# MoFHeka/MeepoEmbedding

Hardware: AMD Instinct MI355X
Metric: key-lookups/sec (higher is better)
Workload: dtype int64 keys / fp32 rows (copy)

## Files before the change

### meepoembedding_amd/csrc/meepo_find.hip

```cpp
#include <hip/hip_runtime.h>
#include <hip/hip_ext.h>

#include <cmath>
#include <cstdlib>
#include <cstring>

#include "meepo_apply_part.h"


namespace mee {


template <int DIM4, int R, int NT>
__device__ __forceinline__ void find_span(const int64_t* __restrict__ tkeys, const f32x4* __restrict__ values, uint64_t nb,
                                          const int64_t* __restrict__ keys, uint64_t n, f32x4* __restrict__ out,
                                          uint8_t* __restrict__ found, float defv, uint32_t dim4_rt, uint32_t* hits,
                                          int64_t* __restrict__ slots_out, uint64_t wave, uint64_t n_waves, int64_t handle_tag = 0) {
    const int lane = threadIdx.x & 63, tile = lane >> 4, tl = lane & 15;
    const uint32_t dim4 = DIM4 ? DIM4 : dim4_rt;
    constexpr int KPW = 4 * R;
    const f32x4 def4 = {defv, defv, defv, defv};

    for (uint64_t base = wave * KPW; base < n; base += n_waves * KPW) {
        int64_t key[R];
        int64_t slot[R];
        uint64_t b[R];
        int64_t kb[R];
        bool inb[R], act[R];
        const int64_t kmine = (lane < KPW && base + lane < n) ? keys[base + lane] : kEmpty;
#pragma unroll
        for (int r = 0; r < R; ++r) {
            const uint64_t i = base + r * 4 + tile;
            inb[r] = i < n;
            key[r] = __shfl(kmine, r * 4 + tile);
            act[r] = inb[r] && !reserved_key(key[r]);
            if constexpr ((NT & 8) != 0) {
                inb[r] = act[r] = act[r] && found[i] == 0;
            }
            if constexpr ((NT & 128) != 0) {
                if (inb[r] && !act[r] && tl == 0 && found) found[i] = 1;
                inb[r] = act[r];
            }
        }
#pragma unroll
        for (int r = 0; r < R; ++r) {
            b[r] = bucket_of(key[r], nb);
            kb[r] = act[r] ? ((NT & 2) ? __builtin_nontemporal_load(&tkeys[b[r] * kW + tl]) : tkeys[b[r] * kW + tl]) : kEmpty;
        }
#pragma unroll
        for (int r = 0; r < R; ++r) slot[r] = tile_probe(tkeys, nb, key[r], act[r], b[r], kb[r], tile, tl);
        if constexpr ((NT & 16) != 0) {
#pragma unroll
            for (int r = 0; r < R; ++r)
                if (slot[r] >= 0 && tl == 0) atomicAdd(&hits[slot[r]], 1u);
        }
        if constexpr (DIM4 != 0) {
            constexpr int C = DIM4 / 16;
            f32x4 row[R][C];
            bool all_hit = true;
#pragma unroll
            for (int r = 0; r < R; ++r) all_hit = all_hit && inb[r] && slot[r] >= 0;
            if (__all(all_hit)) {
#pragma unroll
                for (int r = 0; r < R; ++r)
#pragma unroll
                    for (int c = 0; c < C; ++c)
                        row[r][c] = (NT & 1) ? __builtin_nontemporal_load(&values[(uint64_t)slot[r] * DIM4 + c * 16 + tl]) : values[(uint64_t)slot[r] * DIM4 + c * 16 + tl];
#pragma unroll
                for (int r = 0; r < R; ++r) {
                    const uint64_t i = base + r * 4 + tile;
#pragma unroll
                    for (int c = 0; c < C; ++c) {
                        if constexpr ((NT & 256) != 0) store_bf16x4<(NT & 4) != 0>(out, i * DIM4 + c * 16 + tl, row[r][c]);
                        else { if (NT & 4) out[i * DIM4 + c * 16 + tl] = row[r][c]; else __builtin_nontemporal_store(row[r][c], &out[i * DIM4 + c * 16 + tl]); }
                    }
                }
            } else {
#pragma unroll
                for (int r = 0; r < R; ++r)
#pragma unroll
                    for (int c = 0; c < C; ++c)
                        row[r][c] = slot[r] >= 0 ? ((NT & 1) ? __builtin_nontemporal_load(&values[(uint64_t)slot[r] * DIM4 + c * 16 + tl]) : values[(uint64_t)slot[r] * DIM4 + c * 16 + tl]) : def4;
#pragma unroll
                for (int r = 0; r < R; ++r) {
                    const uint64_t i = base + r * 4 + tile;
                    if (inb[r] && (!(NT & 8) || slot[r] >= 0)) {
#pragma unroll
                        for (int c = 0; c < C; ++c) {
                            if constexpr ((NT & 256) != 0) store_bf16x4<(NT & 4) != 0>(out, i * DIM4 + c * 16 + tl, row[r][c]);
                            else { if (NT & 4) out[i * DIM4 + c * 16 + tl] = row[r][c]; else __builtin_nontemporal_store(row[r][c], &out[i * DIM4 + c * 16 + tl]); }
                        }
                    }
                }
            }
        } else {
#pragma unroll
            for (int r = 0; r < R; ++r) {
                const uint64_t i = base + r * 4 + tile;
                if (inb[r] && (!(NT & 8) || slot[r] >= 0))
                    for (uint32_t c = tl; c < dim4; c += 16) {
                        if constexpr ((NT & 256) != 0) store_bf16x4<true>(out, i * dim4 + c, slot[r] >= 0 ? values[(uint64_t)slot[r] * dim4 + c] : def4);
                        else out[i * dim4 + c] = slot[r] >= 0 ? values[(uint64_t)slot[r] * dim4 + c] : def4;
                    }
            }
        }
        if constexpr ((NT & 64) != 0) {
            const int64_t mine = collect_slots(slot, lane);
            if (lane < KPW && base + lane < n) slots_out[base + lane] = mine >= 0 ? (mine | handle_tag) : mine;
        }
        if (found && !(NT & 32)) {
#pragma unroll
            for (int r = 0; r < R; ++r) {
                const uint64_t i0 = base + r * 4;
                if ((NT & (8 | 128)) == 0 && i0 + 4 <= n && (reinterpret_cast<uintptr_t>(found) & 3) == 0) {
                    const uint64_t m = __ballot(slot[r] >= 0);
                    const uint32_t w = (uint32_t)(m & 1) | ((uint32_t)((m >> 16) & 1) << 8) | ((uint32_t)((m >> 32) & 1) << 16) |
                                       ((uint32_t)((m >> 48) & 1) << 24);
                    if (lane == 0) *reinterpret_cast<uint32_t*>(found + i0) = w;
                } else {
                    const uint64_t i = i0 + tile;
                    if (inb[r] && tl == 0 && (!(NT & 8) || slot[r] >= 0)) found[i] = slot[r] >= 0;
                }
            }
        }
    }
}

template <int DIM4, int R, int NT>
__global__ __launch_bounds__(256) void find_kernel(const int64_t* __restrict__ tkeys, const f32x4* __restrict__ values,
                                                   uint64_t nb, const int64_t* __restrict__ keys, uint64_t n,
                                                   f32x4* __restrict__ out, uint8_t* __restrict__ found, float defv,
                                                   uint32_t dim4_rt, uint32_t* hits, int64_t* __restrict__ slots_out = nullptr, int64_t handle_tag = 0) {
    find_span<DIM4, R, NT>(tkeys, values, nb, keys, n, out, found, defv, dim4_rt, hits, slots_out,
                           (uint64_t)blockIdx.x * (blockDim.x >> 6) + (threadIdx.x >> 6), (uint64_t)gridDim.x * (blockDim.x >> 6), handle_tag);
}

constexpr int kFindPrepareThreads = 256;
constexpr int kFindPrepareR = 2;
template <int DIM4, int R, int NT>
__global__ __launch_bounds__(kFindPrepareThreads, 8) void find_prepare_kernel(const int64_t* __restrict__ tkeys, const f32x4* __restrict__ values, uint64_t nb,
                                                           const int64_t* __restrict__ keys, uint64_t n, f32x4* __restrict__ out,
                                                           uint8_t* __restrict__ found, float defv, uint32_t dim4_rt, int64_t* __restrict__ slots_out,
                                                           int64_t handle_tag, uint32_t part_blocks, uint32_t nbk_hash, uint32_t nbk, uint32_t per_block,
                                                           BucketScratch bk, uint32_t* status, OpCounters* op, uint32_t xcd_split) {
    extern __shared__ unsigned long long part_lds[];
    __shared__ unsigned long long part_wsum[kFindPrepareThreads / 64];
    if (blockIdx.x < part_blocks) {
        PartHot* hot = reinterpret_cast<PartHot*>(part_lds);
        sort_role<kFindPrepareThreads>(keys, (uint32_t)n, nbk_hash, nbk, per_block, blockIdx.x, part_blocks, bk, status, op, reinterpret_cast<uint32_t*>(hot + 1), part_wsum, hot, true, xcd_split);
        return;
    }
    find_span<DIM4, R, NT>(tkeys, values, nb, keys, n, out, found, defv, dim4_rt, nullptr, slots_out,
                           (uint64_t)(blockIdx.x - part_blocks) * (blockDim.x >> 6) + (threadIdx.x >> 6), (uint64_t)(gridDim.x - part_blocks) * (blockDim.x >> 6),
                           handle_tag);
}

constexpr int kMaxFindRequests = 16;
struct FindMany {
    const int64_t* keys[kMaxFindRequests];
    f32x4* out[kMaxFindRequests];
    uint8_t* found[kMaxFindRequests];
    uint64_t n[kMaxFindRequests];
    uint32_t first_block[kMaxFindRequests + 1];
    uint32_t count;
};
template <int DIM4, int R, int NT>
__global__ __launch_bounds__(256) void find_many_kernel(const int64_t* __restrict__ tkeys, const f32x4* __restrict__ values, uint64_t nb,
// ... 351 lines not shown
                pooled_bwd_positions<DIM4, U, C, GROUPED>(tkeys, values, nb, capacity, dim4, kv, pos, inb, wv, handles, handle_tag, member,
                                                          tile, tl, def4, g, grads, weight_grads);
            }
        }
    }
}

}

using namespace mee;

namespace mee {
static bool outputs_rotate(const mee_table* t, const void* d_out, uint64_t bytes) {
    mee_table* m = const_cast<mee_table*>(t);
    const uint64_t p = (uint64_t)(uintptr_t)d_out;
    const uint32_t head = __atomic_load_n(&m->out_ring_head, __ATOMIC_RELAXED);
    if (__atomic_load_n(&m->out_ring_ptr[(head + 7u) & 7u], __ATOMIC_RELAXED) == p) return false;
    const uint32_t slot = __atomic_fetch_add(&m->out_ring_head, 1u, __ATOMIC_RELAXED) & 7u;
    __atomic_store_n(&m->out_ring_ptr[slot], p, __ATOMIC_RELAXED);
    __atomic_store_n(&m->out_ring_bytes[slot], bytes, __ATOMIC_RELAXED);
    uint64_t seen[8], total = 0;
    int distinct = 0;
    for (int i = 0; i < 8; ++i) {
        const uint64_t q = __atomic_load_n(&m->out_ring_ptr[i], __ATOMIC_RELAXED);
        if (!q) continue;
        bool dup = false;
        for (int j = 0; j < distinct; ++j) dup = dup || seen[j] == q;
        if (dup) continue;
        seen[distinct++] = q;
        total += __atomic_load_n(&m->out_ring_bytes[i], __ATOMIC_RELAXED);
    }
    return distinct >= 2 && total > (64ull << 20);
}

template <class F> void with_pooled_shape(uint32_t dim4, size_t n, uint64_t n_bags, F&& f) {
    with_row_shape(dim4, [&](auto d4) {
        if (n / n_bags >= 12) f(d4, std::integral_constant<int, RowShape<d4>::pooled_unroll_1>{}, std::integral_constant<int, 1>{}, grid_for(n_bags, 4, 1u << 20));
        else f(d4, std::integral_constant<int, RowShape<d4>::pooled_unroll_4>{}, std::integral_constant<int, 4>{}, grid_for(n_bags, 16, 1u << 20));
    });
}

int find_plane(const mee_table* t, const float* plane, float miss_value, const int64_t* d_keys, size_t n, float* d_out,
               uint8_t* d_found, void* stream, FindPath path) {
    if (n == 0) return MEE_OK;
    DeviceGuard g(t->device);
    hipStream_t st = as_stream(stream);
    const unsigned fblock = t->find_block == 64 || t->find_block == 128 ? (unsigned)t->find_block : 256u;
    const bool bf16 = path.out_dtype == MEE_DTYPE_BF16;
    const uint64_t out_bytes = (uint64_t)n * t->dim * (bf16 ? 2 : 4);
    const int nt = path.nt >= 0 ? path.nt : t->find_nt >= 0 ? (t->find_nt & 7)
                 : (out_bytes <= kCachedOutputBytes && !outputs_rotate(t, d_out, out_bytes) ? 4 : 0);
    if (path.kind == FindPath::Missing || path.kind == FindPath::CountedMissing) {
        with_value<3, 1>(path.kind == FindPath::CountedMissing ? 3 : 1, [&](auto flags) {
            find_missing_kernel<flags><<<grid_for(n, 256, 8192), 256, 0, st>>>(t->keys, (const float4*)plane, t->nb, t->dim4, d_keys, n, (float4*)d_out, d_found, t->hits);
        });
    } else if (bf16) with_row_shape(t->dim4, [&](auto d4) {
        constexpr int D4 = d4;
        constexpr int R = RowShape<D4>::rows_per_tile;
        const unsigned grid = grid_for(n, (fblock / 64u) * 4u * (unsigned)R, t->find_grid_cap > 0 ? (unsigned)t->find_grid_cap : (1u << 22));
        auto find = [&](auto ntc, int64_t* slots_out, int64_t tag) {
            find_kernel<D4, R, ntc><<<grid, fblock, 0, st>>>(t->keys, (const f32x4*)plane, t->nb, d_keys, n, (f32x4*)d_out, d_found, miss_value, t->dim4, nullptr, slots_out, tag);
        };
        if (path.kind == FindPath::Located) {
            const bool cached_out = t->find_nt >= 0 && (t->find_nt & 4);
            with_value<256 + 68, 256 + 64>(cached_out ? 256 + 68 : 256 + 64, [&](auto ntc) { find(ntc, path.slots_out, handle_tag_of(t)); });
        } else if (path.kind == FindPath::SkipPadding) {
            with_value<256 + 132, 256 + 128>(nt & 4 ? 256 + 132 : 256 + 128, [&](auto ntc) { find(ntc, nullptr, 0); });
        } else {
            with_value<256, 257, 258, 259, 260, 261, 262, 263>(256 | nt, [&](auto ntc) { find(ntc, nullptr, 0); });
        }
    });
    else with_row_shape(t->dim4, [&](auto d4) {
        constexpr int D4 = d4;
        int R = t->find_rounds > 0 ? t->find_rounds : RowShape<D4>::rows_per_tile;
        if (D4 != 16 && R > 4) R = 4;
        if (D4 != 16 && D4 != 32 && R > 2) R = 2;
        R = R >= 8 ? 8 : R >= 4 ? 4 : R >= 2 ? 2 : 1;
        const unsigned grid = grid_for(n, (fblock / 64u) * 4u * (unsigned)R, t->find_grid_cap > 0 ? (unsigned)t->find_grid_cap : (1u << 22));
        auto find = [&](auto rr, auto ntc, unsigned grid_x, unsigned block, uint32_t* hits = nullptr, int64_t* slots_out = nullptr, int64_t tag = 0) {
            find_kernel<D4, rr, ntc><<<grid_x, block, 0, st>>>(t->keys, (const f32x4*)plane, t->nb, d_keys, n, (f32x4*)d_out, d_found, miss_value, t->dim4, hits, slots_out, tag);
        };
        if (path.kind == FindPath::SkipPadding) {
            with_value<2, 1>(R >= 2 ? 2 : 1, [&](auto rr) { with_value<132, 128>(nt & 4 ? 132 : 128, [&](auto ntc) { find(rr, ntc, grid, 256); }); });
        } else if (path.kind == FindPath::Located) {
// ... 29 lines not shown
    if ((flags & MEE_FIND_STREAM_STORES) && (flags & MEE_FIND_CACHED_STORES))
        return fail(MEE_ERR_INVALID_ARG, "%s: MEE_FIND_STREAM_STORES and MEE_FIND_CACHED_STORES exclude each other", name);
    if (flags == MEE_FIND_DEFAULT) return find_plane(t, t->values, t->default_value, d_keys, n, (float*)d_out, d_found, stream, {FindPath::Plain, nullptr, -1, out_dtype});
    const uint64_t out_bytes = (uint64_t)n * t->dim * (out_dtype == MEE_DTYPE_BF16 ? 2 : 4);
    const bool cached_out = (flags & MEE_FIND_CACHED_STORES) ||
                            (!(flags & MEE_FIND_STREAM_STORES) && out_bytes <= kCachedOutputBytes && !outputs_rotate(t, d_out, out_bytes));
    const int nt = (flags & MEE_FIND_STREAM_ROWS ? 1 : 0) | (flags & MEE_FIND_STREAM_BUCKETS ? 2 : 0) | (cached_out ? 4 : 0);
    return find_plane(t, t->values, t->default_value, d_keys, n, (float*)d_out, d_found, stream, {FindPath::Plain, nullptr, nt, out_dtype});
}

int mee_find(const mee_table* t, const int64_t* d_keys, size_t n, float* d_out, uint8_t* d_found, void* stream) {
    MEE_RANGE("mee_find");
    if (!t || (n && (!d_keys || !d_out))) return fail(MEE_ERR_INVALID_ARG, "mee_find: null argument");
    return find_plane(t, t->values, t->default_value, d_keys, n, d_out, d_found, stream);
}

int mee_find_ex(const mee_table* t, const int64_t* d_keys, size_t n, float* d_out, uint8_t* d_found, uint32_t flags, void* stream) {
    MEE_RANGE("mee_find_ex");
    return find_hinted(t, d_keys, n, d_out, d_found, flags, MEE_DTYPE_F32, stream, "mee_find_ex");
}

int mee_find_as(const mee_table* t, const int64_t* d_keys, size_t n, void* d_out, uint32_t out_dtype, uint8_t* d_found, uint32_t flags, void* stream) {
    MEE_RANGE("mee_find_as");
    return find_hinted(t, d_keys, n, d_out, d_found, flags, out_dtype, stream, "mee_find_as");
}

}
namespace mee {
int find_skip_padding(const mee_table* t, const int64_t* d_keys, size_t n, void* d_out, uint8_t* d_found, void* stream, uint32_t out_dtype) {
    if (!t || (n && (!d_keys || !d_out || !d_found))) return fail(MEE_ERR_INVALID_ARG, "find_skip_padding: null argument");
    if (int rc = check_out_dtype(d_out, out_dtype, "find_skip_padding")) return rc;
    return find_plane(t, t->values, t->default_value, d_keys, n, (float*)d_out, d_found, stream, {FindPath::SkipPadding, nullptr, -1, out_dtype});
}
}
extern "C" {

int mee_find_located(const mee_table* t, const int64_t* d_keys, size_t n, float* d_out, uint8_t* d_found, int64_t* d_slots_out, void* stream) {
    MEE_RANGE("mee_find_located");
    if (!t || (n && (!d_keys || !d_out || !d_slots_out))) return fail(MEE_ERR_INVALID_ARG, "mee_find_located: null argument");
    return find_plane(t, t->values, t->default_value, d_keys, n, d_out, d_found, stream, {FindPath::Located, d_slots_out});
}
int mee_find_located_as(const mee_table* t, const int64_t* d_keys, size_t n, void* d_out, uint32_t out_dtype, uint8_t* d_found, int64_t* d_slots_out, void* stream) {
    MEE_RANGE("mee_find_located_as");
    if (!t || (n && (!d_keys || !d_out || !d_slots_out))) return fail(MEE_ERR_INVALID_ARG, "mee_find_located_as: null argument");
    if (int rc = check_out_dtype(d_out, out_dtype, "mee_find_located_as")) return rc;
    return find_plane(t, t->values, t->default_value, d_keys, n, (float*)d_out, d_found, stream, {FindPath::Located, d_slots_out, -1, out_dtype});
}

int mee_find_many(const mee_table* t, const mee_find_request* reqs, uint32_t count, void* stream) {
    MEE_RANGE("mee_find_many");
    if (!t || !reqs) return fail(MEE_ERR_INVALID_ARG, "mee_find_many: null argument");
    if (count == 0) return MEE_OK;
    if (count > (uint32_t)kMaxFindRequests) return fail(MEE_ERR_INVALID_ARG, "mee_find_many: %u requests (at most %d per call)", count, kMaxFindRequests);
    FindMany m{};
    const int R = with_row_shape(t->dim4, [](auto d4) { return RowShape<d4>::rows_per_tile; });
    uint64_t blocks = 0, out_bytes = 0;
    uint32_t used = 0;
    for (uint32_t q = 0; q < count; ++q) {
        if (reqs[q].n == 0) continue;
        if (!reqs[q].d_keys || !reqs[q].d_out) return fail(MEE_ERR_INVALID_ARG, "mee_find_many: request %u has a null buffer", q);
        m.keys[used] = reqs[q].d_keys; m.out[used] = (f32x4*)reqs[q].d_out; m.found[used] = reqs[q].d_found; m.n[used] = reqs[q].n;
        m.first_block[used] = (uint32_t)blocks;
        blocks += (reqs[q].n + 16ull * R - 1) / (16ull * R);
        out_bytes += (uint64_t)reqs[q].n * t->dim * 4;
        ++used;
    }
// ... 207 lines not shown
```

### meepoembedding_amd/csrc/meepo_host.h

```cpp
#pragma once
#include <hip/hip_runtime.h>
#include <cstdarg>
#include <cstdio>
#include <type_traits>

#include "../../include/meepo_embedding.h"

namespace mee {

char* last_error_buf();

inline int fail(int code, const char* fmt, ...) {
    va_list ap;
    va_start(ap, fmt);
    vsnprintf(last_error_buf(), 512, fmt, ap);
    va_end(ap);
    return code;
}

#define MEE_HIP(expr)                                                                                     \
    do {                                                                                                  \
        hipError_t e_ = (expr);                                                                           \
        if (e_ != hipSuccess)                                                                             \
            return ::mee::fail(e_ == hipErrorOutOfMemory ? MEE_ERR_OUT_OF_MEMORY : MEE_ERR_HIP,           \
// ... 19 lines not shown
    OpRange& operator=(const OpRange&) = delete;
};
#define MEE_RANGE(name) ::mee::OpRange mee_range_(name)

struct DeviceGuard {
    int prev = -1;
    bool switched = false;
    hipError_t err = hipSuccess;
    explicit DeviceGuard(int device) {
        err = hipGetDevice(&prev);
        if (err == hipSuccess && prev != device) { err = hipSetDevice(device); switched = (err == hipSuccess); }
    }
    ~DeviceGuard() { if (switched) (void)hipSetDevice(prev); }
};

struct TableView {
    int device;
    const int64_t* keys;
    const float* values;
    uint64_t nb;
    uint32_t dim, dim4;
    float default_value;
    uint64_t generation;
    float *s1, *s2;
    uint32_t optimizer;
    uint32_t initializer;
    float init_scale, init_acc;
    uint64_t init_seed;
    uint32_t* status;
    uint32_t* hits;
};
TableView table_view(const mee_table* t);
int find_skip_padding(const mee_table* t, const int64_t* d_keys, size_t n, void* d_out, uint8_t* d_found, void* stream, uint32_t out_dtype = MEE_DTYPE_F32);

struct GroupDesc {
    const int64_t* tkeys;
    float4* values;
    float4* s1;
    float4* s2;
    uint64_t nb;
    float defv;
    uint32_t pad;
};
struct GroupInit {
    uint64_t init_seed;
    uint32_t* status;
    uint32_t* hits;
    uint32_t initializer, optimizer;
    float init_scale, init_acc;
};
constexpr int kGroupSlotBits = 48;
constexpr uint32_t kMaxGroupTables = 1024;

inline unsigned grid_for(size_t work_items, unsigned per_block, unsigned cap) {
    size_t g = (work_items + per_block - 1) / per_block;
    if (g < 1) g = 1;
    if (g > cap) g = cap;
    return (unsigned)g;
}

constexpr uint64_t kCachedOutputBytes = 128ull << 20;

template <class F> decltype(auto) with_row_shape(uint32_t dim4, F&& f) {
    if (dim4 == 16) return f(std::integral_constant<int, 16>{});
    if (dim4 == 32) return f(std::integral_constant<int, 32>{});
    return f(std::integral_constant<int, 0>{});
// ... 33 lines not shown
```

### meepoembedding_amd/csrc/meepo_sharded.hip

```cpp
#include <hip/hip_runtime.h>
#include <rccl/rccl.h>

#include <dlfcn.h>

#include <atomic>
#include <cmath>
#include <cstdlib>
#include <cstring>
#include <mutex>
#include <new>
#include <mutex>
#include <unordered_set>
#include <vector>

#include "meepo_device.h"
#include "meepo_host.h"

namespace mee {

struct RcclApi {
    void* handle = nullptr;
    ncclResult_t (*GetUniqueId)(ncclUniqueId*) = nullptr;
    ncclResult_t (*CommInitRank)(ncclComm_t*, int, ncclUniqueId, int) = nullptr;
    ncclResult_t (*CommDestroy)(ncclComm_t) = nullptr;
// ... 40 lines not shown
    });
    return api.handle ? &api : nullptr;
}
static const char* rccl_load_error() {
    (void)rccl_api();
    return rccl_state().error[0] ? rccl_state().error : "RCCL could not be loaded (librccl.so.1 not found or incomplete)";
}

#define MEE_NCCL(api, expr)                                                                                        \
    do {                                                                                                           \
        ncclResult_t r_ = (expr);                                                                                  \
        if (r_ != ncclSuccess)                                                                                     \
            return ::mee::fail(MEE_ERR_RCCL, "%s failed: %s (%s:%d)", #expr, (api)->GetErrorString(r_), __FILE__, __LINE__); \
    } while (0)

__device__ __forceinline__ uint64_t seg_base(const uint64_t* __restrict__ counts, uint32_t p) {
    uint64_t b = 0;
    for (uint32_t q = 0; q < p; ++q) b += counts[q];
    return b;
}

__global__ __launch_bounds__(256) void shard_pad_keys_kernel(const int64_t* __restrict__ send_keys, const uint64_t* __restrict__ counts,
                                                             uint64_t cap, int64_t* __restrict__ pad, uint32_t* status) {
    const uint32_t p = blockIdx.y;
    const uint64_t cnt = counts[p], take = cnt < cap ? cnt : cap, b0 = seg_base(counts, p);
    int64_t* __restrict__ dst = pad + (uint64_t)p * cap;
    for (uint64_t j = blockIdx.x * (uint64_t)blockDim.x + threadIdx.x; j < cap; j += (uint64_t)gridDim.x * blockDim.x)
        dst[j] = j < take ? send_keys[b0 + j] : kEmpty;
    if (cnt > cap && blockIdx.x == 0 && threadIdx.x == 0) atomicOr(status, 1u);
}

__global__ __launch_bounds__(256) void shard_pack_rows_kernel(const float4* __restrict__ rows, const int64_t* __restrict__ perm,
                                                              const uint64_t* __restrict__ counts, uint64_t cap ,
                                                              uint32_t dim4, float4* __restrict__ dst) {
    const int lane = threadIdx.x & 63, tile = lane >> 4, tl = lane & 15;
    const uint32_t p = blockIdx.y;
    const uint64_t cnt = counts[p], take = (cap && cnt > cap) ? cap : cnt, b0 = seg_base(counts, p);
    const uint64_t off = cap ? (uint64_t)p * cap : b0;
    const uint64_t wave = (uint64_t)blockIdx.x * (blockDim.x >> 6) + (threadIdx.x >> 6), n_waves = (uint64_t)gridDim.x * (blockDim.x >> 6);
    for (uint64_t j0 = wave * 4; j0 < take; j0 += n_waves * 4) {
        const uint64_t j = j0 + tile;
        if (j >= take) continue;
        const uint64_t src = (uint64_t)perm[b0 + j] * dim4;
        for (uint32_t c = tl; c < dim4; c += 16) dst[(off + j) * dim4 + c] = rows[src + c];
    }
}

template <bool BF16> struct RowGroup { using type = float4; };
template <> struct RowGroup<true> { using type = u32x2; };
template <bool BF16>
__global__ __launch_bounds__(256) void shard_return_kernel(const typename RowGroup<BF16>::type* __restrict__ back_rows, const uint8_t* __restrict__ back_found,
                                                           const int64_t* __restrict__ perm, const uint64_t* __restrict__ counts,
                                                           uint64_t cap , uint32_t dim4, typename RowGroup<BF16>::type* __restrict__ out,
                                                           uint8_t* __restrict__ found, float defv, const int64_t* __restrict__ send_keys) {
    const int lane = threadIdx.x & 63, tile = lane >> 4, tl = lane & 15;
    const uint32_t p = blockIdx.y;
    const uint64_t cnt = counts[p], take = (cap && cnt > cap) ? cap : cnt, b0 = seg_base(counts, p);
    const uint64_t off = cap ? (uint64_t)p * cap : b0;
    const uint64_t wave = (uint64_t)blockIdx.x * (blockDim.x >> 6) + (threadIdx.x >> 6), n_waves = (uint64_t)gridDim.x * (blockDim.x >> 6);
    typename RowGroup<BF16>::type def4;
    if constexpr (BF16) def4 = bf16x4_of(defv, defv, defv, defv); else def4 = make_float4(defv, defv, defv, defv);
    for (uint64_t j0 = wave * 4; j0 < cnt; j0 += n_waves * 4) {
        const uint64_t j = j0 + tile;
        if (j >= cnt) continue;
        const uint64_t dstp = (uint64_t)perm[b0 + j];
        const bool sent = j < take && !(cap && reserved_key(send_keys[b0 + j]));
        if (out && (back_rows || !sent))
            for (uint32_t c = tl; c < dim4; c += 16) out[dstp * dim4 + c] = sent ? back_rows[(off + j) * dim4 + c] : def4;
        if (found && (back_found || !sent) && tl == 0) found[dstp] = sent ? back_found[off + j] : (uint8_t)0;
    }
}

template <bool BF16>
__global__ __launch_bounds__(256) void shard_expand_kernel(const typename RowGroup<BF16>::type* __restrict__ urows, const uint8_t* __restrict__ ufound,
                                                           const int64_t* __restrict__ inverse, uint64_t n, uint32_t dim4,
                                                           typename RowGroup<BF16>::type* __restrict__ out, uint8_t* __restrict__ found) {
    const int lane = threadIdx.x & 63, tile = lane >> 4, tl = lane & 15;
    const uint64_t wave = (uint64_t)blockIdx.x * (blockDim.x >> 6) + (threadIdx.x >> 6), n_waves = (uint64_t)gridDim.x * (blockDim.x >> 6);
    for (uint64_t i0 = wave * 16; i0 < n; i0 += n_waves * 16) {
        uint64_t u[4];
#pragma unroll
        for (int q = 0; q < 4; ++q) { const uint64_t i = i0 + q * 4 + tile; u[q] = i < n ? (uint64_t)inverse[i] : 0ull; }
        for (uint32_t c = tl; c < dim4; c += 16) {
            typename RowGroup<BF16>::type r[4];
#pragma unroll
            for (int q = 0; q < 4; ++q) r[q] = urows[u[q] * dim4 + c];
#pragma unroll
            for (int q = 0; q < 4; ++q) {
                const uint64_t i = i0 + q * 4 + tile;
// ... 81 lines not shown
};

namespace mee {

static void sharded_free(mee_sharded* c) {
    void* dev[] = {c->send_keys, c->perm, c->pad_keys, c->counts, c->d_recv_counts, c->send_rows, c->back_rows, c->back_found,
                   c->recv_keys, c->recv_rows, c->recv_found, c->recv_found2, c->status, c->wire_rows, c->uniq, c->inverse, c->urows, c->ufound,
                   c->img_keys, c->keys2, c->perm2, c->counts2, c->rows2};
    for (void* p : dev) if (p) (void)hipFree(p);
    if (c->h_counts) (void)hipHostFree(c->h_counts);
    if (c->h_counts2) (void)hipHostFree(c->h_counts2);
    if (c->router) mee_router_destroy(c->router);
    if (c->sub_router) mee_router_destroy(c->sub_router);
    if (c->dd) mee_table_destroy(c->dd);
}

static int ensure_send_rows(mee_sharded* c) {
    if (c->send_rows) return MEE_OK;
    MEE_HIP(hipMalloc((void**)&c->send_rows, c->send_slots * (uint64_t)c->dim * 4));
    return MEE_OK;
}

static int ensure_wire_rows(mee_sharded* c) {
    if (c->wire_rows) return MEE_OK;
    MEE_HIP(hipMalloc(&c->wire_rows, c->recv_slots * (uint64_t)c->dim * 2));
    return MEE_OK;
}

struct Leg {
    const void* send; void* recv;
    size_t elems;
    size_t elem_bytes;
    ncclDataType_t dt;
};

static std::mutex g_abort_mu;
static std::unordered_set<void*> g_aborted;
static bool comm_is_aborted(void* comm) { std::lock_guard<std::mutex> lk(g_abort_mu); return g_aborted.count(comm) != 0; }
static void abort_comm(RcclApi* api, ncclComm_t comm) {
    {
        std::lock_guard<std::mutex> lk(g_abort_mu);
        if (!g_aborted.insert((void*)comm).second) return;
    }
    if (api->CommAbort) (void)api->CommAbort(comm);
}

static int rccl_failed(mee_sharded* c, RcclApi* api, ncclResult_t err, const char* what) {
    c->dead = true;
    abort_comm(api, c->comm);
    return fail(MEE_ERR_RCCL, "%s failed: %s — the communicator was aborted (and thereby freed: do not destroy it), every sharded context on it is unusable", what, api->GetErrorString(err));
}

static int exchange(mee_sharded* c, const Leg* legs, int n_legs, bool reverse, hipStream_t st) {
    RcclApi* api = rccl_api();
    if (!api) return fail(MEE_ERR_RCCL, "%s", rccl_load_error());
    const std::vector<size_t>& sc = reverse ? c->rcount : c->scount;
    const std::vector<size_t>& sd = reverse ? c->rdisp : c->sdisp;
    const std::vector<size_t>& rc = reverse ? c->scount : c->rcount;
    const std::vector<size_t>& rd = reverse ? c->sdisp : c->rdisp;
    for (int l = 0; l < n_legs; ++l) {
        const size_t row = legs[l].elems * legs[l].elem_bytes;
        if (sc[c->rank])
            MEE_HIP(hipMemcpyAsync((char*)legs[l].recv + rd[c->rank] * row, (const char*)legs[l].send + sd[c->rank] * row, sc[c->rank] * row,
                                   hipMemcpyDeviceToDevice, st));
    }
    if (c->G == 1) return MEE_OK;
    ncclResult_t first_err = api->GroupStart();
    if (first_err != ncclSuccess) return rccl_failed(c, api, first_err, "ncclGroupStart");
    for (uint32_t p = 0; p < c->G && first_err == ncclSuccess; ++p) {
        if (p == c->rank) continue;
        for (int l = 0; l < n_legs && first_err == ncclSuccess; ++l) {
            const size_t row = legs[l].elems * legs[l].elem_bytes;
            if (sc[p]) { first_err = api->Send((const char*)legs[l].send + sd[p] * row, sc[p] * legs[l].elems, legs[l].dt, (int)p, c->comm, st); c->sent_bytes += sc[p] * row; }
            if (rc[p] && first_err == ncclSuccess) { first_err = api->Recv((char*)legs[l].recv + rd[p] * row, rc[p] * legs[l].elems, legs[l].dt, (int)p, c->comm, st); c->recv_bytes += rc[p] * row; }
        }
    }
    const ncclResult_t end_err = api->GroupEnd();
    if (first_err != ncclSuccess) return rccl_failed(c, api, first_err, "ncclSend/ncclRecv");
    if (end_err != ncclSuccess) return rccl_failed(c, api, end_err, "ncclGroupEnd");
    return MEE_OK;
}

static int route(mee_sharded* c, const int64_t* d_keys, size_t n, hipStream_t st, const int64_t** keys_to_send, uint64_t* r_total, bool skip_padding = false) {
    if (int rc = skip_padding ? mee_partition_padded(c->router, d_keys, n, c->send_keys, c->counts, c->perm, st)
                              : mee_partition(c->router, d_keys, n, c->send_keys, c->counts, c->perm, st)) return rc;
    if (c->cap) {
        const dim3 grid(grid_for(c->cap, 256, 256), c->G);
        shard_pad_keys_kernel<<<grid, 256, 0, st>>>(c->send_keys, c->counts, c->cap, c->pad_keys, c->status);
        MEE_HIP(hipGetLastError());
        *keys_to_send = c->pad_keys;
        *r_total = (uint64_t)c->G * c->cap;
        return MEE_OK;
    }
    RcclApi* api = rccl_api();
    if (!api) return fail(MEE_ERR_RCCL, "%s", rccl_load_error());
    MEE_HIP(hipMemcpyAsync(c->d_recv_counts + c->rank, c->counts + c->rank, 8, hipMemcpyDeviceToDevice, st));
    if (c->G > 1) {
        ncclResult_t first_err = api->GroupStart();
        if (first_err != ncclSuccess) return rccl_failed(c, api, first_err, "ncclGroupStart");
        for (uint32_t p = 0; p < c->G && first_err == ncclSuccess; ++p) {
            if (p == c->rank) continue;
            first_err = api->Send(c->counts + p, 1, ncclUint64, (int)p, c->comm, st);
            c->sent_bytes += 8;
            if (first_err == ncclSuccess) { first_err = api->Recv(c->d_recv_counts + p, 1, ncclUint64, (int)p, c->comm, st); c->recv_bytes += 8; }
        }
        const ncclResult_t end_err = api->GroupEnd();
        if (first_err != ncclSuccess || end_err != ncclSuccess) return rccl_failed(c, api, first_err != ncclSuccess ? first_err : end_err, "counts exchange");
    }
    MEE_HIP(hipMemcpyAsync(c->h_counts, c->counts, c->G * 8, hipMemcpyDeviceToHost, st));
    MEE_HIP(hipMemcpyAsync(c->h_counts + c->G, c->d_recv_counts, c->G * 8, hipMemcpyDeviceToHost, st));
    MEE_HIP(hipStreamSynchronize(st));
    size_t s_acc = 0, r_acc = 0;
    for (uint32_t p = 0; p < c->G; ++p) {
        c->scount[p] = (size_t)c->h_counts[p]; c->sdisp[p] = s_acc; s_acc += c->scount[p];
        c->rcount[p] = (size_t)c->h_counts[c->G + p]; c->rdisp[p] = r_acc; r_acc += c->rcount[p];
    }
    if (r_acc > c->recv_slots) {
        c->dead = true;
        abort_comm(api, c->comm);
        return fail(MEE_ERR_BATCH_TOO_LARGE, "%llu keys arrive at this shard, more than G x max_batch = %llu: a rank exceeded the max_batch the ranks agreed on",
                    (unsigned long long)r_acc, (unsigned long long)c->recv_slots);
    }
    *keys_to_send = c->send_keys;
    *r_total = r_acc;
    return MEE_OK;
}

static int pack_rows(mee_sharded* c, const float* d_rows, hipStream_t st) {
    if (int rc = ensure_send_rows(c)) return rc;
    const dim3 grid(grid_for(c->max_batch / c->G + 64, 16, 4096), c->G);
    shard_pack_rows_kernel<<<grid, 256, 0, st>>>((const float4*)d_rows, c->perm, c->counts, c->cap, c->dim4, (float4*)c->send_rows);
    MEE_HIP(hipGetLastError());
    return MEE_OK;
}

static int give_back(mee_sharded* c, bool rows, void* d_out, uint8_t* d_found, hipStream_t st, bool bf16 = false) {
    Leg legs[2];
    int nl = 0;
    if (rows) legs[nl++] = bf16 ? Leg{c->cold ? c->wire_rows : (void*)c->recv_rows, c->back_rows, c->dim, 2, ncclBfloat16}
                                : Leg{c->recv_rows, c->back_rows, c->dim, 4, ncclFloat};
    legs[nl++] = Leg{c->recv_found, c->back_found, 1, 1, ncclUint8};
    if (int rc = exchange(c, legs, nl, true, st)) return rc;
    const dim3 grid(grid_for(c->max_batch / c->G + 64, 16, 4096), c->G);
    if (bf16)
        shard_return_kernel<true><<<grid, 256, 0, st>>>(rows ? (const u32x2*)c->back_rows : nullptr, c->back_found, c->perm, c->counts, c->cap, c->dim4,
                                                        (u32x2*)d_out, d_found, c->defv, c->send_keys);
    else
        shard_return_kernel<false><<<grid, 256, 0, st>>>(rows ? (const float4*)c->back_rows : nullptr, c->back_found, c->perm, c->counts, c->cap, c->dim4,
                                                         (float4*)d_out, d_found, c->defv, c->send_keys);
    MEE_HIP(hipGetLastError());
    return MEE_OK;
}

static int check_call(const mee_sharded* c, size_t n, const char* name) {
    if (!c) return fail(MEE_ERR_INVALID_ARG, "%s: null context", name);
    if (c->dead || comm_is_aborted((void*)c->comm)) return fail(MEE_ERR_RCCL, "%s: an earlier RCCL error aborted this context's communicator", name);
    if (n > c->max_batch) return fail(MEE_ERR_BATCH_TOO_LARGE, "%s: n=%zu exceeds the context's max_batch=%llu", name, n, (unsigned long long)c->max_batch);
    return MEE_OK;
}

static int push(mee_sharded* c, const int64_t* d_keys, const float* d_rows, size_t n, hipStream_t st, uint64_t* r_total, bool skip_padding = false) {
    const int64_t* ks = nullptr;
    if (int rc = route(c, d_keys, n, st, &ks, r_total, skip_padding)) return rc;
    Leg legs[2];
    int nl = 0;
    legs[nl++] = Leg{ks, c->recv_keys, 1, 8, ncclInt64};
    if (d_rows) {
        if (int rc = pack_rows(c, d_rows, st)) return rc;
        legs[nl++] = Leg{c->send_rows, c->recv_rows, c->dim, 4, ncclFloat};
    }
    return exchange(c, legs, nl, false, st);
}

static int hot_has_room(mee_sharded* c, uint64_t n, void* stream, bool* room) {
    if (c->hot_ub + n > c->hot_limit) {
        size_t sz = 0;
        if (int rc = mee_size(c->local, &sz, stream)) return rc;
        c->hot_ub = sz;
    }
    *room = c->hot_ub + n <= c->hot_limit;
    return MEE_OK;
}

static int owner_lookup(mee_sharded* c, uint64_t rt, bool insert_missing, void* stream, bool bf16 = false) {
    if (rt == 0) return MEE_OK;
    if (!c->cold && insert_missing) {
        for (uint64_t s = 0; s < rt; s += c->local_max_batch) {
            const uint64_t m = rt - s < c->local_max_batch ? rt - s : c->local_max_batch;
            if (int rc = bf16 ? mee_find_or_insert_as(c->local, c->recv_keys + s, m, (uint16_t*)c->recv_rows + s * c->dim, MEE_DTYPE_BF16, c->recv_found + s, stream)
                              : mee_find_or_insert(c->local, c->recv_keys + s, m, c->recv_rows + s * c->dim, c->recv_found + s, stream)) return rc;
        }
        return MEE_OK;
    }
    if (bf16 && !c->cold)
        return c->cap ? find_skip_padding(c->local, c->recv_keys, rt, c->recv_rows, c->recv_found, stream, MEE_DTYPE_BF16)
                      : mee_find_as(c->local, c->recv_keys, rt, c->recv_rows, MEE_DTYPE_BF16, c->recv_found, MEE_FIND_DEFAULT, stream);
    if (int rc = c->cap ? find_skip_padding(c->local, c->recv_keys, rt, c->recv_rows, c->recv_found, stream)
                        : mee_find(c->local, c->recv_keys, rt, c->recv_rows, c->recv_found, stream)) return rc;
    if (!c->cold) return MEE_OK;
    if (int rc = mee_find_missing(c->cold, c->recv_keys, rt, c->recv_rows, c->recv_found, stream)) return rc;
    for (uint64_t s = 0; insert_missing && s < rt; s += c->local_max_batch) {
        const uint64_t m = rt - s < c->local_max_batch ? rt - s : c->local_max_batch;
// ... 231 lines not shown
        if (he == hipSuccess && ne == ncclSuccess) he = hipMemcpy(c->h_counts, c->d_recv_counts, c->G * 8, hipMemcpyDeviceToHost);
        if (he != hipSuccess) rc = fail(MEE_ERR_HIP, "mee_sharded_create_ex: %s", hipGetErrorString(he));
        else if (ne != ncclSuccess) rc = fail(MEE_ERR_RCCL, "mee_sharded_create_ex: ncclAllReduce failed: %s", api->GetErrorString(ne));
        else
            for (uint32_t p = 0; p < c->G; ++p)
                if (c->h_counts[p] != c->h_counts[c->rank]) {
                    rc = fail(MEE_ERR_INVALID_ARG, "mee_sharded_create_ex: rank %u was created with another max_batch / pad_slack than rank %u (all ranks must agree)", p, c->rank);
                    break;
                }
    }
    if (rc != MEE_OK) { sharded_free(c); delete c; return rc; }
    *out = c;
    return MEE_OK;
}

int mee_sharded_create(mee_table* local, void* nccl_comm, uint64_t max_batch, double pad_slack, mee_sharded** out) {
    MEE_RANGE("mee_sharded_create");
    mee_sharded_options o;
    memset(&o, 0, sizeof o);
    o.struct_size = sizeof o; o.max_batch = max_batch; o.pad_slack = pad_slack;
    return mee_sharded_create_ex(local, nccl_comm, &o, out);
}

static int sharded_lookup(mee_sharded* c, const int64_t* d_keys, size_t n, void* d_out, uint32_t out_dtype, uint8_t* d_found, void* stream, bool insert_missing,
                          const char* name) {
    if (int rc = check_call(c, n, name)) return rc;
    if (n && (!d_keys || !d_out)) return fail(MEE_ERR_INVALID_ARG, "%s: null argument", name);
    if (int rc = check_out_dtype(d_out, out_dtype, name)) return rc;
    const bool bf16 = out_dtype == MEE_DTYPE_BF16;
    DeviceGuard g(c->device);
    hipStream_t st = (hipStream_t)stream;
    uint64_t rt = 0;
    if (bf16 && c->cold) if (int rc = ensure_wire_rows(c)) return rc;
    if (!c->dedup) {
        if (int rc = push(c, d_keys, nullptr, n, st, &rt)) return rc;
        if (int rc = owner_lookup(c, rt, insert_missing, stream, bf16)) return rc;
        return give_back(c, true, d_out, d_found, st, bf16);
    }
    if (n) if (int rc = mee_dedup_keys(c->dd, d_keys, n, c->uniq, c->inverse, (int64_t)c->max_batch, stream)) return rc;
    if (int rc = push(c, c->uniq, nullptr, n, st, &rt, true)) return rc;
    if (int rc = owner_lookup(c, rt, insert_missing, stream, bf16)) return rc;
    if (int rc = give_back(c, true, c->urows, c->ufound, st, bf16)) return rc;
    if (n && bf16) {
        shard_fill_row_bf16_kernel<<<1, 256, 0, st>>>((u32x2*)c->urows + c->max_batch * (uint64_t)c->dim4, c->dim4, c->defv, c->ufound + c->max_batch);
        shard_expand_kernel<true><<<grid_for(n, 64, 1u << 16), 256, 0, st>>>((const u32x2*)c->urows, c->ufound, c->inverse, n, c->dim4, (u32x2*)d_out, d_found);
        MEE_HIP(hipGetLastError());
    } else if (n) {
        shard_expand_kernel<false><<<grid_for(n, 64, 1u << 16), 256, 0, st>>>((const float4*)c->urows, c->ufound, c->inverse, n, c->dim4, (float4*)d_out, d_found);
        MEE_HIP(hipGetLastError());
    }
    return MEE_OK;
}

int mee_sharded_find(mee_sharded* c, const int64_t* d_keys, size_t n, float* d_out, uint8_t* d_found, void* stream) {
    MEE_RANGE("mee_sharded_find");
    return sharded_lookup(c, d_keys, n, d_out, MEE_DTYPE_F32, d_found, stream, false, "mee_sharded_find");
}
int mee_sharded_find_or_insert(mee_sharded* c, const int64_t* d_keys, size_t n, float* d_out, uint8_t* d_found, void* stream) {
    MEE_RANGE("mee_sharded_find_or_insert");
    return sharded_lookup(c, d_keys, n, d_out, MEE_DTYPE_F32, d_found, stream, true, "mee_sharded_find_or_insert");
}
int mee_sharded_find_as(mee_sharded* c, const int64_t* d_keys, size_t n, void* d_out, uint32_t out_dtype, uint8_t* d_found, void* stream) {
    MEE_RANGE("mee_sharded_find_as");
    return sharded_lookup(c, d_keys, n, d_out, out_dtype, d_found, stream, false, "mee_sharded_find_as");
}
int mee_sharded_find_or_insert_as(mee_sharded* c, const int64_t* d_keys, size_t n, void* d_out, uint32_t out_dtype, uint8_t* d_found, void* stream) {
    MEE_RANGE("mee_sharded_find_or_insert_as");
    return sharded_lookup(c, d_keys, n, d_out, out_dtype, d_found, stream, true, "mee_sharded_find_or_insert_as");
}

int mee_sharded_insert(mee_sharded* c, const int64_t* d_keys, const float* d_values, size_t n, void* stream) {
    MEE_RANGE("mee_sharded_insert");
    if (int rc = check_call(c, n, "mee_sharded_insert")) return rc;
    if (n && (!d_keys || !d_values)) return fail(MEE_ERR_INVALID_ARG, "mee_sharded_insert: null argument");
    DeviceGuard g(c->device);
// ... 121 lines not shown
```

Baseline: 7.821 billion.

## Serve self-owned shard keys in place with a scattering find kernel

In sharded find, keys owned by the local rank are no longer copied into the receive buffer, looked up there, and copied back before being scattered by the return kernel. A new find_scatter_kernel looks up the local segment directly from the partitioned send keys and writes rows straight to their final output positions through the permutation. The exchange legs skip the self memcpy, receive displacements exclude the self segment, and the return kernel skips the self partition. This removes two device-to-device copies and one scatter pass for the local share. In exchange it adds more bookkeeping in route and in the displacement arrays, and the rows are now written through an indirect scatter.

```diff
diff --git a/meepoembedding_amd/csrc/meepo_find.hip b/meepoembedding_amd/csrc/meepo_find.hip
--- a/meepoembedding_amd/csrc/meepo_find.hip
+++ b/meepoembedding_amd/csrc/meepo_find.hip
@@ -15,7 +15,8 @@
 __device__ __forceinline__ void find_span(const int64_t* __restrict__ tkeys, const f32x4* __restrict__ values, uint64_t nb,
                                           const int64_t* __restrict__ keys, uint64_t n, f32x4* __restrict__ out,
                                           uint8_t* __restrict__ found, float defv, uint32_t dim4_rt, uint32_t* hits,
-                                          int64_t* __restrict__ slots_out, uint64_t wave, uint64_t n_waves, int64_t handle_tag = 0) {
+                                          int64_t* __restrict__ slots_out, uint64_t wave, uint64_t n_waves, int64_t handle_tag = 0,
+                                          const int64_t* __restrict__ dst = nullptr, uint64_t n_act = 0) {
     const int lane = threadIdx.x & 63, tile = lane >> 4, tl = lane & 15;
     const uint32_t dim4 = DIM4 ? DIM4 : dim4_rt;
     constexpr int KPW = 4 * R;
@@ -28,12 +29,16 @@
         int64_t kb[R];
         bool inb[R], act[R];
         const int64_t kmine = (lane < KPW && base + lane < n) ? keys[base + lane] : kEmpty;
+        uint64_t od[R];
+        int64_t dmine = 0;
+        if constexpr ((NT & 512) != 0) dmine = (lane < KPW && base + lane < n) ? dst[base + lane] : 0;
 #pragma unroll
         for (int r = 0; r < R; ++r) {
             const uint64_t i = base + r * 4 + tile;
             inb[r] = i < n;
             key[r] = __shfl(kmine, r * 4 + tile);
             act[r] = inb[r] && !reserved_key(key[r]);
+            if constexpr ((NT & 512) != 0) { od[r] = (uint64_t)__shfl(dmine, r * 4 + tile); act[r] = act[r] && i < n_act; }
             if constexpr ((NT & 8) != 0) {
                 inb[r] = act[r] = act[r] && found[i] == 0;
             }
@@ -68,7 +73,7 @@
                         row[r][c] = (NT & 1) ? __builtin_nontemporal_load(&values[(uint64_t)slot[r] * DIM4 + c * 16 + tl]) : values[(uint64_t)slot[r] * DIM4 + c * 16 + tl];
 #pragma unroll
                 for (int r = 0; r < R; ++r) {
-                    const uint64_t i = base + r * 4 + tile;
+                    const uint64_t i = (NT & 512) ? od[r] : base + r * 4 + tile;
 #pragma unroll
                     for (int c = 0; c < C; ++c) {
                         if constexpr ((NT & 256) != 0) store_bf16x4<(NT & 4) != 0>(out, i * DIM4 + c * 16 + tl, row[r][c]);
@@ -83,7 +88,7 @@
                         row[r][c] = slot[r] >= 0 ? ((NT & 1) ? __builtin_nontemporal_load(&values[(uint64_t)slot[r] * DIM4 + c * 16 + tl]) : values[(uint64_t)slot[r] * DIM4 + c * 16 + tl]) : def4;
 #pragma unroll
                 for (int r = 0; r < R; ++r) {
-                    const uint64_t i = base + r * 4 + tile;
+                    const uint64_t i = (NT & 512) ? od[r] : base + r * 4 + tile;
                     if (inb[r] && (!(NT & 8) || slot[r] >= 0)) {
 #pragma unroll
                         for (int c = 0; c < C; ++c) {
@@ -96,7 +101,7 @@
         } else {
 #pragma unroll
             for (int r = 0; r < R; ++r) {
-                const uint64_t i = base + r * 4 + tile;
+                const uint64_t i = (NT & 512) ? od[r] : base + r * 4 + tile;
                 if (inb[r] && (!(NT & 8) || slot[r] >= 0))
                     for (uint32_t c = tl; c < dim4; c += 16) {
                         if constexpr ((NT & 256) != 0) store_bf16x4<true>(out, i * dim4 + c, slot[r] >= 0 ? values[(uint64_t)slot[r] * dim4 + c] : def4);
@@ -112,13 +117,13 @@
 #pragma unroll
             for (int r = 0; r < R; ++r) {
                 const uint64_t i0 = base + r * 4;
-                if ((NT & (8 | 128)) == 0 && i0 + 4 <= n && (reinterpret_cast<uintptr_t>(found) & 3) == 0) {
+                if ((NT & (8 | 128 | 512)) == 0 && i0 + 4 <= n && (reinterpret_cast<uintptr_t>(found) & 3) == 0) {
                     const uint64_t m = __ballot(slot[r] >= 0);
                     const uint32_t w = (uint32_t)(m & 1) | ((uint32_t)((m >> 16) & 1) << 8) | ((uint32_t)((m >> 32) & 1) << 16) |
                                        ((uint32_t)((m >> 48) & 1) << 24);
                     if (lane == 0) *reinterpret_cast<uint32_t*>(found + i0) = w;
                 } else {
-                    const uint64_t i = i0 + tile;
+                    const uint64_t i = (NT & 512) ? od[r] : i0 + tile;
                     if (inb[r] && tl == 0 && (!(NT & 8) || slot[r] >= 0)) found[i] = slot[r] >= 0;
                 }
             }
@@ -133,6 +138,19 @@
                                                    uint32_t dim4_rt, uint32_t* hits, int64_t* __restrict__ slots_out = nullptr, int64_t handle_tag = 0) {
     find_span<DIM4, R, NT>(tkeys, values, nb, keys, n, out, found, defv, dim4_rt, hits, slots_out,
                            (uint64_t)blockIdx.x * (blockDim.x >> 6) + (threadIdx.x >> 6), (uint64_t)gridDim.x * (blockDim.x >> 6), handle_tag);
+}
+
+template <int DIM4, int R, int NT>
+__global__ __launch_bounds__(256) void find_scatter_kernel(const int64_t* __restrict__ tkeys, const f32x4* __restrict__ values, uint64_t nb,
+                                                           const int64_t* __restrict__ seg_keys, const int64_t* __restrict__ perm,
+                                                           const uint64_t* __restrict__ counts, uint32_t p, uint64_t cap, f32x4* __restrict__ out,
+                                                           uint8_t* __restrict__ found, float defv, uint32_t dim4_rt) {
+    static_assert((NT & 512) != 0, "find_scatter_kernel is the scattering find");
+    uint64_t b0 = 0;
+    for (uint32_t q = 0; q < p; ++q) b0 += counts[q];
+    const uint64_t cnt = counts[p], take = (cap && cnt > cap) ? cap : cnt;
+    find_span<DIM4, R, NT>(tkeys, values, nb, seg_keys + b0, cnt, out, found, defv, dim4_rt, nullptr, nullptr,
+                           (uint64_t)blockIdx.x * (blockDim.x >> 6) + (threadIdx.x >> 6), (uint64_t)gridDim.x * (blockDim.x >> 6), 0, perm + b0, take);
 }
 
 constexpr int kFindPrepareThreads = 256;
@@ -550,6 +568,9 @@
     }
     return distinct >= 2 && total > (64ull << 20);
 }
+static int default_nt(const mee_table* t, const void* d_out, uint64_t out_bytes) {
+    return t->find_nt >= 0 ? (t->find_nt & 7) : (out_bytes <= kCachedOutputBytes && !outputs_rotate(t, d_out, out_bytes) ? 4 : 0);
+}
 
 template <class F> void with_pooled_shape(uint32_t dim4, size_t n, uint64_t n_bags, F&& f) {
     with_row_shape(dim4, [&](auto d4) {
@@ -566,8 +587,7 @@
     const unsigned fblock = t->find_block == 64 || t->find_block == 128 ? (unsigned)t->find_block : 256u;
     const bool bf16 = path.out_dtype == MEE_DTYPE_BF16;
     const uint64_t out_bytes = (uint64_t)n * t->dim * (bf16 ? 2 : 4);
-    const int nt = path.nt >= 0 ? path.nt : t->find_nt >= 0 ? (t->find_nt & 7)
-                 : (out_bytes <= kCachedOutputBytes && !outputs_rotate(t, d_out, out_bytes) ? 4 : 0);
+    const int nt = path.nt >= 0 ? path.nt : default_nt(t, d_out, out_bytes);
     if (path.kind == FindPath::Missing || path.kind == FindPath::CountedMissing) {
         with_value<3, 1>(path.kind == FindPath::CountedMissing ? 3 : 1, [&](auto flags) {
             find_missing_kernel<flags><<<grid_for(n, 256, 8192), 256, 0, st>>>(t->keys, (const float4*)plane, t->nb, t->dim4, d_keys, n, (float4*)d_out, d_found, t->hits);
@@ -663,6 +683,22 @@
     if (int rc = check_out_dtype(d_out, out_dtype, "find_skip_padding")) return rc;
     return find_plane(t, t->values, t->default_value, d_keys, n, (float*)d_out, d_found, stream, {FindPath::SkipPadding, nullptr, -1, out_dtype});
 }
+int find_scatter_segment(const mee_table* t, const int64_t* d_seg_keys, const int64_t* d_perm, const uint64_t* d_counts, uint32_t p, uint64_t cap, size_t n_bound,
+                         size_t n_out, void* d_out, uint8_t* d_found, void* stream, uint32_t out_dtype) {
+    if (n_bound == 0) return MEE_OK;
+    if (!t || !d_seg_keys || !d_perm || !d_counts || !d_out) return fail(MEE_ERR_INVALID_ARG, "find_scatter_segment: null argument");
+    if (int rc = check_out_dtype(d_out, out_dtype, "find_scatter_segment")) return rc;
+    DeviceGuard g(t->device);
+    const bool bf16 = out_dtype == MEE_DTYPE_BF16;
+    const int nt = default_nt(t, d_out, (uint64_t)n_out * t->dim * (bf16 ? 2 : 4)) & 4;
+    with_row_shape(t->dim4, [&](auto d4) { with_value<256, 0>(bf16 ? 256 : 0, [&](auto wide) { with_value<4, 0>(nt, [&](auto ntc) {
+        constexpr int R = RowShape<d4>::rows_per_tile;
+        find_scatter_kernel<d4, R, 512 | wide | ntc><<<grid_for(n_bound, 16u * R, 1u << 22), 256, 0, as_stream(stream)>>>(
+            t->keys, (const f32x4*)t->values, t->nb, d_seg_keys, d_perm, d_counts, p, cap, (f32x4*)d_out, d_found, t->default_value, t->dim4);
+    }); }); });
+    MEE_HIP(hipGetLastError());
+    return MEE_OK;
+}
 }
 extern "C" {
 
diff --git a/meepoembedding_amd/csrc/meepo_host.h b/meepoembedding_amd/csrc/meepo_host.h
--- a/meepoembedding_amd/csrc/meepo_host.h
+++ b/meepoembedding_amd/csrc/meepo_host.h
@@ -75,6 +75,8 @@
 };
 TableView table_view(const mee_table* t);
 int find_skip_padding(const mee_table* t, const int64_t* d_keys, size_t n, void* d_out, uint8_t* d_found, void* stream, uint32_t out_dtype = MEE_DTYPE_F32);
+int find_scatter_segment(const mee_table* t, const int64_t* d_seg_keys, const int64_t* d_perm, const uint64_t* d_counts, uint32_t p, uint64_t cap, size_t n_bound,
+                         size_t n_out, void* d_out, uint8_t* d_found, void* stream, uint32_t out_dtype = MEE_DTYPE_F32);
 
 struct GroupDesc {
     const int64_t* tkeys;
diff --git a/meepoembedding_amd/csrc/meepo_sharded.hip b/meepoembedding_amd/csrc/meepo_sharded.hip
--- a/meepoembedding_amd/csrc/meepo_sharded.hip
+++ b/meepoembedding_amd/csrc/meepo_sharded.hip
@@ -96,11 +96,12 @@
 
 __global__ __launch_bounds__(256) void shard_pack_rows_kernel(const float4* __restrict__ rows, const int64_t* __restrict__ perm,
                                                               const uint64_t* __restrict__ counts, uint64_t cap ,
-                                                              uint32_t dim4, float4* __restrict__ dst) {
+                                                              uint32_t dim4, float4* __restrict__ dst, uint32_t self_p, float4* __restrict__ self_dst) {
     const int lane = threadIdx.x & 63, tile = lane >> 4, tl = lane & 15;
     const uint32_t p = blockIdx.y;
     const uint64_t cnt = counts[p], take = (cap && cnt > cap) ? cap : cnt, b0 = seg_base(counts, p);
-    const uint64_t off = cap ? (uint64_t)p * cap : b0;
+    uint64_t off = cap ? (uint64_t)p * cap : b0;
+    if (p == self_p) { dst = self_dst; off = 0; }
     const uint64_t wave = (uint64_t)blockIdx.x * (blockDim.x >> 6) + (threadIdx.x >> 6), n_waves = (uint64_t)gridDim.x * (blockDim.x >> 6);
     for (uint64_t j0 = wave * 4; j0 < take; j0 += n_waves * 4) {
         const uint64_t j = j0 + tile;
@@ -116,9 +117,11 @@
 __global__ __launch_bounds__(256) void shard_return_kernel(const typename RowGroup<BF16>::type* __restrict__ back_rows, const uint8_t* __restrict__ back_found,
                                                            const int64_t* __restrict__ perm, const uint64_t* __restrict__ counts,
                                                            uint64_t cap , uint32_t dim4, typename RowGroup<BF16>::type* __restrict__ out,
-                                                           uint8_t* __restrict__ found, float defv, const int64_t* __restrict__ send_keys) {
+                                                           uint8_t* __restrict__ found, float defv, const int64_t* __restrict__ send_keys,
+                                                           uint32_t skip_p ) {
     const int lane = threadIdx.x & 63, tile = lane >> 4, tl = lane & 15;
     const uint32_t p = blockIdx.y;
+    if (p == skip_p) return;
     const uint64_t cnt = counts[p], take = (cap && cnt > cap) ? cap : cnt, b0 = seg_base(counts, p);
     const uint64_t off = cap ? (uint64_t)p * cap : b0;
     const uint64_t wave = (uint64_t)blockIdx.x * (blockDim.x >> 6) + (threadIdx.x >> 6), n_waves = (uint64_t)gridDim.x * (blockDim.x >> 6);
@@ -266,6 +269,7 @@
     size_t elems;
     size_t elem_bytes;
     ncclDataType_t dt;
+    bool self_copy = true;
 };
 
 static std::mutex g_abort_mu;
@@ -294,7 +298,7 @@
     const std::vector<size_t>& rd = reverse ? c->sdisp : c->rdisp;
     for (int l = 0; l < n_legs; ++l) {
         const size_t row = legs[l].elems * legs[l].elem_bytes;
-        if (sc[c->rank])
+        if (legs[l].self_copy && sc[c->rank])
             MEE_HIP(hipMemcpyAsync((char*)legs[l].recv + rd[c->rank] * row, (const char*)legs[l].send + sd[c->rank] * row, sc[c->rank] * row,
                                    hipMemcpyDeviceToDevice, st));
     }
@@ -315,15 +319,17 @@
     return MEE_OK;
 }
 
-static int route(mee_sharded* c, const int64_t* d_keys, size_t n, hipStream_t st, const int64_t** keys_to_send, uint64_t* r_total, bool skip_padding = false) {
+static int route(mee_sharded* c, const int64_t* d_keys, size_t n, hipStream_t st, const int64_t** keys_to_send, uint64_t* r_total, bool skip_padding = false,
+                 bool self_in_place = false) {
     if (int rc = skip_padding ? mee_partition_padded(c->router, d_keys, n, c->send_keys, c->counts, c->perm, st)
                               : mee_partition(c->router, d_keys, n, c->send_keys, c->counts, c->perm, st)) return rc;
     if (c->cap) {
         const dim3 grid(grid_for(c->cap, 256, 256), c->G);
         shard_pad_keys_kernel<<<grid, 256, 0, st>>>(c->send_keys, c->counts, c->cap, c->pad_keys, c->status);
         MEE_HIP(hipGetLastError());
+        for (uint32_t p = 0; p < c->G; ++p) c->rdisp[p] = (size_t)(self_in_place && p > c->rank ? p - 1 : p) * c->cap;
         *keys_to_send = c->pad_keys;
-        *r_total = (uint64_t)c->G * c->cap;
+        *r_total = (uint64_t)(c->G - (self_in_place ? 1 : 0)) * c->cap;
         return MEE_OK;
     }
     RcclApi* api = rccl_api();
@@ -347,7 +353,8 @@
     size_t s_acc = 0, r_acc = 0;
     for (uint32_t p = 0; p < c->G; ++p) {
         c->scount[p] = (size_t)c->h_counts[p]; c->sdisp[p] = s_acc; s_acc += c->scount[p];
-        c->rcount[p] = (size_t)c->h_counts[c->G + p]; c->rdisp[p] = r_acc; r_acc += c->rcount[p];
+        c->rcount[p] = (size_t)c->h_counts[c->G + p]; c->rdisp[p] = r_acc;
+        if (!(self_in_place && p == c->rank)) r_acc += c->rcount[p];
     }
     if (r_acc > c->recv_slots) {
         c->dead = true;
@@ -363,25 +370,28 @@
 static int pack_rows(mee_sharded* c, const float* d_rows, hipStream_t st) {
     if (int rc = ensure_send_rows(c)) return rc;
     const dim3 grid(grid_for(c->max_batch / c->G + 64, 16, 4096), c->G);
-    shard_pack_rows_kernel<<<grid, 256, 0, st>>>((const float4*)d_rows, c->perm, c->counts, c->cap, c->dim4, (float4*)c->send_rows);
+    shard_pack_rows_kernel<<<grid, 256, 0, st>>>((const float4*)d_rows, c->perm, c->counts, c->cap, c->dim4, (float4*)c->send_rows, c->rank,
+                                                 (float4*)(c->recv_rows + c->rdisp[c->rank] * (uint64_t)c->dim));
     MEE_HIP(hipGetLastError());
     return MEE_OK;
 }
 
-static int give_back(mee_sharded* c, bool rows, void* d_out, uint8_t* d_found, hipStream_t st, bool bf16 = false) {
+static int give_back(mee_sharded* c, bool rows, void* d_out, uint8_t* d_found, hipStream_t st, bool bf16 = false, bool self_served = false) {
+    if (self_served && c->G == 1) return MEE_OK;
     Leg legs[2];
     int nl = 0;
-    if (rows) legs[nl++] = bf16 ? Leg{c->cold ? c->wire_rows : (void*)c->recv_rows, c->back_rows, c->dim, 2, ncclBfloat16}
-                                : Leg{c->recv_rows, c->back_rows, c->dim, 4, ncclFloat};
-    legs[nl++] = Leg{c->recv_found, c->back_found, 1, 1, ncclUint8};
+    if (rows) legs[nl++] = bf16 ? Leg{c->cold ? c->wire_rows : (void*)c->recv_rows, c->back_rows, c->dim, 2, ncclBfloat16, !self_served}
+                                : Leg{c->recv_rows, c->back_rows, c->dim, 4, ncclFloat, !self_served};
+    legs[nl++] = Leg{c->recv_found, c->back_found, 1, 1, ncclUint8, !self_served};
     if (int rc = exchange(c, legs, nl, true, st)) return rc;
+    const uint32_t skip_p = self_served ? c->rank : ~0u;
     const dim3 grid(grid_for(c->max_batch / c->G + 64, 16, 4096), c->G);
     if (bf16)
         shard_return_kernel<true><<<grid, 256, 0, st>>>(rows ? (const u32x2*)c->back_rows : nullptr, c->back_found, c->perm, c->counts, c->cap, c->dim4,
-                                                        (u32x2*)d_out, d_found, c->defv, c->send_keys);
+                                                        (u32x2*)d_out, d_found, c->defv, c->send_keys, skip_p);
     else
         shard_return_kernel<false><<<grid, 256, 0, st>>>(rows ? (const float4*)c->back_rows : nullptr, c->back_found, c->perm, c->counts, c->cap, c->dim4,
-                                                         (float4*)d_out, d_found, c->defv, c->send_keys);
+                                                         (float4*)d_out, d_found, c->defv, c->send_keys, skip_p);
     MEE_HIP(hipGetLastError());
     return MEE_OK;
 }
@@ -393,15 +403,16 @@
     return MEE_OK;
 }
 
-static int push(mee_sharded* c, const int64_t* d_keys, const float* d_rows, size_t n, hipStream_t st, uint64_t* r_total, bool skip_padding = false) {
+static int push(mee_sharded* c, const int64_t* d_keys, const float* d_rows, size_t n, hipStream_t st, uint64_t* r_total, bool skip_padding = false,
+                bool self_in_place = false) {
     const int64_t* ks = nullptr;
-    if (int rc = route(c, d_keys, n, st, &ks, r_total, skip_padding)) return rc;
+    if (int rc = route(c, d_keys, n, st, &ks, r_total, skip_padding, self_in_place)) return rc;
     Leg legs[2];
     int nl = 0;
-    legs[nl++] = Leg{ks, c->recv_keys, 1, 8, ncclInt64};
+    legs[nl++] = Leg{ks, c->recv_keys, 1, 8, ncclInt64, !self_in_place};
     if (d_rows) {
         if (int rc = pack_rows(c, d_rows, st)) return rc;
-        legs[nl++] = Leg{c->send_rows, c->recv_rows, c->dim, 4, ncclFloat};
+        legs[nl++] = Leg{c->send_rows, c->recv_rows, c->dim, 4, ncclFloat, false};
     }
     return exchange(c, legs, nl, false, st);
 }
@@ -699,15 +710,23 @@
     hipStream_t st = (hipStream_t)stream;
     uint64_t rt = 0;
     if (bf16 && c->cold) if (int rc = ensure_wire_rows(c)) return rc;
+    const bool in_place = !insert_missing && !c->cold;
+    auto serve_self = [&](void* out, uint8_t* found) -> int {
+        if (!in_place) return MEE_OK;
+        const size_t bound = c->cap ? (n < c->cap ? n : (size_t)c->cap) : c->scount[c->rank];
+        return find_scatter_segment(c->local, c->send_keys, c->perm, c->counts, c->rank, c->cap, bound, n, out, found, stream, out_dtype);
+    };
     if (!c->dedup) {
-        if (int rc = push(c, d_keys, nullptr, n, st, &rt)) return rc;
+        if (int rc = push(c, d_keys, nullptr, n, st, &rt, false, in_place)) return rc;
         if (int rc = owner_lookup(c, rt, insert_missing, stream, bf16)) return rc;
-        return give_back(c, true, d_out, d_found, st, bf16);
+        if (int rc = serve_self(d_out, d_found)) return rc;
+        return give_back(c, true, d_out, d_found, st, bf16, in_place);
     }
     if (n) if (int rc = mee_dedup_keys(c->dd, d_keys, n, c->uniq, c->inverse, (int64_t)c->max_batch, stream)) return rc;
-    if (int rc = push(c, c->uniq, nullptr, n, st, &rt, true)) return rc;
+    if (int rc = push(c, c->uniq, nullptr, n, st, &rt, true, in_place)) return rc;
     if (int rc = owner_lookup(c, rt, insert_missing, stream, bf16)) return rc;
-    if (int rc = give_back(c, true, c->urows, c->ufound, st, bf16)) return rc;
+    if (int rc = serve_self(c->urows, c->ufound)) return rc;
+    if (int rc = give_back(c, true, c->urows, c->ufound, st, bf16, in_place)) return rc;
     if (n && bf16) {
         shard_fill_row_bf16_kernel<<<1, 256, 0, st>>>((u32x2*)c->urows + c->max_batch * (uint64_t)c->dim4, c->dim4, c->defv, c->ufound + c->max_batch);
         shard_expand_kernel<true><<<grid_for(n, 64, 1u << 16), 256, 0, st>>>((const u32x2*)c->urows, c->ufound, c->inverse, n, c->dim4, (u32x2*)d_out, d_found);
```

After: 7.814 billion. Within noise of the previous version (-0.1%).
